# lab-incert/peba1

Measured on AMD Instinct MI355X. Metric: bootstrapped gates/sec (blind rotations/s) over the PEBA1 match path, and end-to-end match ms, higher is better.
Workload: dtype u32

## Files before the change

### peba1_amd/csrc/kernels.hip

```cpp
#include <type_traits>

#include "kernels.hpp"
#include "ntt_wave.hpp"

namespace tfhe_hip {

namespace {

__device__ __forceinline__ PrimeCtx make_ctx(int q, const uint32_t *tw, int n_ring) {
    PrimeCtx c;
    c.P = q ? NTT_P1 : NTT_P0;
    c.pinv = q ? NTT_PINV1 : NTT_PINV0;
    c.rmod = q ? NTT_R[1] : NTT_R[0];
    c.wf = tw + (size_t)(q * 2 + 0) * n_ring;
    c.wi = tw + (size_t)(q * 2 + 1) * n_ring;
    const uint4 *quads = reinterpret_cast<const uint4 *>(tw + (size_t)4 * n_ring);
    c.qf = quads + (size_t)(q * 2 + 0) * (n_ring / 2);
    c.qi = quads + (size_t)(q * 2 + 1) * (n_ring / 2);
    c.dtab = nullptr;
    c.fw1 = nullptr;
    c.fw2 = nullptr;
    return c;
}

// ... 10 lines not shown
    for (int r = 0; r < REGS; ++r) y[r] = mont_redc(acc[r], c.P, c.pinv);
    WaveNtt<LOGN>::inverse(y, c, scr, lane);
}

template <int LOGN>
__global__ __launch_bounds__(64) void bk_transform_kernel(const int32_t *__restrict__ raw, uint32_t *__restrict__ img,
                                                          const uint32_t *__restrict__ tw, int nw,
                                                          uint32_t scale0, uint32_t scale1) {
    using NTT = WaveNtt<LOGN>;
    constexpr int N = NTT::N, REGS = NTT::REGS;
    __shared__ __align__(16) uint32_t scr[NTT::SCRATCH_WORDS];
    const int lane = threadIdx.x;
    const int q = blockIdx.y;
    const int poly = blockIdx.x;
    const int X = poly / nw, w = poly % nw;
    const PrimeCtx c = make_ctx(q, tw, N);
    const uint32_t scale = q ? scale1 : scale0;
    const int32_t *src = raw + (size_t)poly * N;
    int32_t x[REGS];
#pragma unroll
    for (int r = 0; r < REGS; ++r) x[r] = src[r * 64 + lane] % (int32_t)c.P;
    NTT::forward(x, c, scr, lane);
    uint4 *dst = reinterpret_cast<uint4 *>(img + ((size_t)(X * 2 + q) * nw + w) * N) + lane;
#pragma unroll
    for (int g = 0; g < REGS / 4; ++g) {
        uint32_t v[4];
#pragma unroll
        for (int e = 0; e < 4; ++e) {
            int32_t m = x[4 * g + e] % (int32_t)c.P;
            if (m < 0) m += (int32_t)c.P;
            v[e] = (uint32_t)((uint64_t)(uint32_t)m * scale % c.P);
        }
        dst[g * 64] = make_uint4(v[0], v[1], v[2], v[3]);
    }
}

template <int LOGN>
__global__ __launch_bounds__(128) void negacyclic_kernel(const int32_t *__restrict__ ip, const uint32_t *__restrict__ img,
                                                         const uint32_t *__restrict__ tw, int32_t *__restrict__ res) {
    using NTT = WaveNtt<LOGN>;
    constexpr int N = NTT::N, REGS = NTT::REGS;
    __shared__ __align__(16) uint32_t lds_scr[2][NTT::SCRATCH_WORDS];
    const int tid = threadIdx.x;
    const int q = __builtin_amdgcn_readfirstlane(tid >> 6);
    const int lane = tid & 63;
    const PrimeCtx c = make_ctx(q, tw, N);
    uint32_t *scr = lds_scr[q];
    const int32_t *src = ip + (size_t)blockIdx.x * N;
    int32_t x[REGS];
#pragma unroll
    for (int r = 0; r < REGS; ++r) x[r] = src[r * 64 + lane];
    NTT::forward(x, c, scr, lane);
    const uint4 *bp = reinterpret_cast<const uint4 *>(img + (size_t)(blockIdx.x * 2 + q) * N) + lane;
    int64_t acc[REGS];
#pragma unroll
    for (int g = 0; g < REGS / 4; ++g) {
        const uint4 b = bp[g * 64];
        acc[4 * g + 0] = (int64_t)x[4 * g + 0] * (int32_t)b.x;
        acc[4 * g + 1] = (int64_t)x[4 * g + 1] * (int32_t)b.y;
        acc[4 * g + 2] = (int64_t)x[4 * g + 2] * (int32_t)b.z;
        acc[4 * g + 3] = (int64_t)x[4 * g + 3] * (int32_t)b.w;
    }
    int32_t y[REGS];
    finish_inverse<LOGN>(acc, y, c, scr, lane);
#pragma unroll
    for (int r = 0; r < REGS; ++r) scr[r * 64 + lane] = (uint32_t)y[r];
    __syncthreads();
    if (q == 0) {
        const uint32_t *oscr = lds_scr[1];
#pragma unroll
        for (int r = 0; r < REGS; ++r)
            res[(size_t)blockIdx.x * N + r * 64 + lane] = (int32_t)crt_signed_to_torus(y[r], (int32_t)oscr[r * 64 + lane]);
    }
}

template <int LOGN, int THREADS>
__device__ __forceinline__ void prelude_modswitch(const DevParams &p, const RotDesc &rd, const int32_t *__restrict__ pool,
                                                  uint16_t *lds_bar, int tid) {
    const int32_t *A = pool + (size_t)rd.slot_a * p.ct_stride;
    const int32_t *B = pool + (size_t)rd.slot_b * p.ct_stride;
    if (rd.slot_c < 0) {
        for (int i = tid; i <= p.n; i += THREADS) {
            uint32_t t = (uint32_t)rd.sa * (uint32_t)A[i] + (uint32_t)rd.sb * (uint32_t)B[i];
            if (i == p.n) t += (uint32_t)rd.c0;
            lds_bar[i] = (uint16_t)((t + (1u << (30 - LOGN))) >> (31 - LOGN));
        }
    } else {
        const int32_t *C = pool + (size_t)rd.slot_c * p.ct_stride;
        for (int i = tid; i <= p.n; i += THREADS) {
            uint32_t t = (uint32_t)rd.sa * (uint32_t)A[i] + (uint32_t)rd.sb * (uint32_t)B[i] + (uint32_t)rd.sc * (uint32_t)C[i];
            if (i == p.n) t += (uint32_t)rd.c0;
            lds_bar[i] = (uint16_t)((t + (1u << (30 - LOGN))) >> (31 - LOGN));
        }
    }
}

struct ClockProbe {
    unsigned long long c0 = 0, r0 = 0;
    bool on = false;
    __device__ __forceinline__ void begin(const DevParams &p) {
        on = p.clock_acc != nullptr && blockIdx.x % 61 == 0 && threadIdx.x == 0;
        if (on) { c0 = __builtin_amdgcn_s_memtime(); r0 = __builtin_amdgcn_s_memrealtime(); }
    }
    __device__ __forceinline__ void end(const DevParams &p) {
        if (on) {
            atomicAdd(&p.clock_acc[0], __builtin_amdgcn_s_memtime() - c0);
            atomicAdd(&p.clock_acc[1], __builtin_amdgcn_s_memrealtime() - r0);
        }
    }
};

template <int LOGN>
__device__ __forceinline__ uint32_t testvector_coef(int j, int barb, int32_t mu) {
    constexpr int N = 1 << LOGN;
    const int idx = (j + barb) & (2 * N - 1);
    return (idx & N) ? (uint32_t)(-mu) : (uint32_t)mu;
}

template <int LOGN>
__device__ __forceinline__ uint32_t lut_coef(const int32_t *__restrict__ v, int j, int barb) {
    constexpr int N = 1 << LOGN;
    const int idx = (j + barb) & (2 * N - 1);
    const uint32_t w = (uint32_t)v[idx & (N - 1)];
    return (idx & N) ? 0u - w : w;
}

__device__ __forceinline__ const int32_t *lut_of(const DevParams &p, const RotDesc &rd) {
    return rd.lut >= 0 ? p.luts + (size_t)rd.lut * LUT_STRIDE : nullptr;
}

template <int LOGN>
__device__ __forceinline__ uint32_t body_coef(const int32_t *__restrict__ lut, int j, int barb, int32_t mu) {
    return lut ? lut_coef<LOGN>(lut, j, barb) : testvector_coef<LOGN>(j, barb, mu);
}

template <int LOGN>
struct AccLds {
    static constexpr int N = 1 << LOGN;
    uint32_t w[2][3 * N];
    __device__ __forceinline__ void set(int u, int j, uint32_t v) {
        w[u][j] = v; w[u][N + j] = 0u - v; w[u][2 * N + j] = v;
    }
    __device__ __forceinline__ uint32_t get(int u, int j) const { return w[u][j]; }
    template <int REGS>
    __device__ __forceinline__ void rotated_difference(uint32_t (&D)[REGS], int u, int lane, int abar, uint32_t offset) const {
        const uint32_t base = (uint32_t)(lane - abar) & (uint32_t)(2 * N - 1);
        const uint32_t *own_neg = w[u] + N + lane;
        const uint32_t *rot = w[u] + base;
#pragma unroll
        for (int r = 0; r < REGS; ++r) D[r] = (rot[r * 64] + own_neg[r * 64] + offset) ^ offset;
    }
};

template <int LOGN, bool FRESH, bool TABLE, bool LDSTW = false, bool PROGRESS = false, int V = 0>
__device__ __forceinline__ void forward_poly(const DevParams &p, const DevKey &key, const PrimeCtx &c,
                                             const AccLds<LOGN> &lds_acc, uint32_t *scr,
                                             int lane, int q, int i, int u, int abar, bool swap_outputs,
                                             int64_t (&acc0)[WaveNtt<LOGN>::REGS], int64_t (&acc1)[WaveNtt<LOGN>::REGS],
                                             const typename WaveNtt<LOGN>::FwdTw0 &t0, int jbegin = 0, int jend = -1) {
    using NTT = WaveNtt<LOGN>;
    constexpr int N = NTT::N, REGS = NTT::REGS, G4 = REGS / 4;
    uint32_t Dk[REGS];
    lds_acc.template rotated_difference<REGS>(Dk, u, lane, abar, p.decomp_offset);
    const int o0 = swap_outputs ? N / 4 : 0, o1 = N / 4 - o0;
    const int width = p.Bgbit;
    auto row = [&](int jj, auto first) {
        const int prow = u * p.l + jj;
        const uint4 *bp = reinterpret_cast<const uint4 *>(
                              key.bk_img + ((size_t)((size_t)i * p.kpl + prow) * 2 + q) * 2 * N) + lane;
        uint4 b0[G4], b1[G4];
#pragma unroll
        for (int g = 0; g < G4; ++g) b0[g] = bp[o0 + g * 64];
#pragma unroll
        for (int g = 0; g < G4; ++g) b1[g] = bp[o1 + g * 64];
        const int shift = 32 - (jj + 1) * width;
        int32_t x[REGS];
        NTT::template forward_digits<TABLE, LDSTW>(x, Dk, shift, width, c, scr, lane, t0);
#pragma unroll
        for (int g = 0; g < G4; ++g) {
            const int32_t bb0[4] = {(int32_t)b0[g].x, (int32_t)b0[g].y, (int32_t)b0[g].z, (int32_t)b0[g].w};
#pragma unroll
            for (int e = 0; e < 4; ++e) {
                const int r = 4 * g + e;
                if constexpr (decltype(first)::value) acc0[r] = (int64_t)x[r] * bb0[e];
                else acc0[r] += (int64_t)x[r] * bb0[e];
            }
        }
#pragma unroll
        for (int g = 0; g < G4; ++g) {
            const int32_t bb1[4] = {(int32_t)b1[g].x, (int32_t)b1[g].y, (int32_t)b1[g].z, (int32_t)b1[g].w};
#pragma unroll
            for (int e = 0; e < 4; ++e) {
                const int r = 4 * g + e;
                if constexpr (decltype(first)::value) acc1[r] = (int64_t)x[r] * bb1[e];
                else acc1[r] += (int64_t)x[r] * bb1[e];
            }
        }
    };
    if (jend < 0) jend = p.l;
    row(jbegin, std::integral_constant<bool, FRESH>{});
#pragma unroll 1
    for (int jj = jbegin + 1; jj < jend; ++jj) {
        if constexpr (PROGRESS) {
            if (jj == jbegin + 1) __builtin_amdgcn_s_setprio(1);
            else __builtin_amdgcn_s_setprio(2);
        }
        row(jj, std::false_type{});
    }
}

template <int LOGN, int THREADS, typename AccT>
__device__ __forceinline__ void extract_outputs(const DevParams &p, const RotDesc &rd, const AccT &acc,
                                                int32_t *__restrict__ u_buf, int tid) {
    constexpr int N = 1 << LOGN;
    const ExtractSpec &xs = p.specs[rd.spec & XS_ENTRY_MASK];
    const int wanted = rd.spec >> XS_WANTED_SHIFT, nout = xs.nout;
    for (int m = 0; m < nout; ++m) {
        if (!((wanted >> m) & 1)) continue;
        int32_t *u = u_buf + (size_t)(rd.u_index + m) * p.u_stride;
        const int nt = xs.ntaps[m];
        for (int i = tid; i < N; i += THREADS) {
            uint32_t sum = 0;
            for (int t = 0; t < nt; ++t) {
                const int d = xs.index[m][t] - i;
                const uint32_t a = acc.get(0, d & (N - 1));
                sum += (uint32_t)xs.weight[m][t] * (d < 0 ? 0u - a : a);
            }
            u[i] = (int32_t)sum;
        }
        if (tid == 0) {
            uint32_t b = (uint32_t)xs.out_c0[m];
            for (int t = 0; t < nt; ++t) b += (uint32_t)xs.weight[m][t] * acc.get(1, xs.index[m][t]);
            u[N] = (int32_t)b;
        }
    }
}

template <int LOGN, int THREADS, typename AccT>
__device__ __forceinline__ void extract_sample(const DevParams &p, const RotDesc &rd,
                                               const AccT &acc,
                                               int32_t *__restrict__ u_buf, int32_t *__restrict__ acc_dbg, int tid) {
    constexpr int N = 1 << LOGN;
    if (rd.spec >= 0) {
        extract_outputs<LOGN, THREADS>(p, rd, acc, u_buf, tid);
    } else {
        int32_t *u = u_buf + (size_t)rd.u_index * p.u_stride;
        for (int j = tid; j < N; j += THREADS)
            u[j] = (int32_t)(j == 0 ? acc.get(0, 0) : 0u - acc.get(0, N - j));
        if (tid == 0) u[N] = (int32_t)acc.get(1, 0);
    }
    if (acc_dbg) {
        int32_t *d = acc_dbg + (size_t)blockIdx.x * 2 * N;
        for (int j = tid; j < 2 * N; j += THREADS) d[j] = (int32_t)acc.get(j >> LOGN, j & (N - 1));
    }
}

template <int LOGN>
__global__ __launch_bounds__(128) void blind_rotate2_kernel(DevParams p, DevKey key, const int32_t *__restrict__ pool,
                                                           const RotDesc *__restrict__ rots,
                                                           int32_t *__restrict__ u_buf, int32_t *__restrict__ acc_dbg) {
    using NTT = WaveNtt<LOGN>;
    constexpr int N = NTT::N, REGS = NTT::REGS;
    __shared__ __align__(16) AccLds<LOGN> lds_acc;
    __shared__ __align__(16) uint32_t lds_scr[2][NTT::SCRATCH_WORDS];
    __shared__ uint16_t lds_bar[1024 + 8];

    const int tid = threadIdx.x;
    const int q = __builtin_amdgcn_readfirstlane(tid >> 6);
    const int lane = tid & 63;
    const PrimeCtx c = make_ctx(q, key.tw, N);
    uint32_t *scr = lds_scr[q];
    const RotDesc rd = rots[blockIdx.x];
    const int n = p.n;

    prelude_modswitch<LOGN, 128>(p, rd, pool, lds_bar, tid);
    __syncthreads();
    {
        const int barb = lds_bar[n];
        const int32_t *lut = lut_of(p, rd);
#pragma unroll
        for (int r = 0; r < REGS; ++r) {
            const int j = r * 64 + lane;
            lds_acc.set(q, j, q == 0 ? 0u : body_coef<LOGN>(lut, j, barb, p.mu));
        }
    }
    __syncthreads();

    typename NTT::FwdTw0 t0;
    t0.load(c, lane);
    for (int i = 0; i < n; ++i) {
        const int abar = __builtin_amdgcn_readfirstlane((int)lds_bar[i]);
        if (abar == 0) continue;

        int64_t acc0[REGS], acc1[REGS];
        forward_poly<LOGN, true, false>(p, key, c, lds_acc, scr, lane, q, i, 0, abar, false, acc0, acc1, t0);
        forward_poly<LOGN, false, false>(p, key, c, lds_acc, scr, lane, q, i, 1, abar, false, acc0, acc1, t0);

        int32_t y0[REGS], y1[REGS];
        finish_inverse<LOGN>(acc0, y0, c, scr, lane);
        finish_inverse<LOGN>(acc1, y1, c, scr, lane);

        const uint32_t *oscr = lds_scr[1 - q];
        if (q == 0) {
#pragma unroll
            for (int r = 0; r < REGS; ++r) scr[r * 64 + lane] = (uint32_t)y1[r];
            __syncthreads();
#pragma unroll
            for (int r = 0; r < REGS; ++r)
                lds_acc.set(0, r * 64 + lane, lds_acc.get(0, r * 64 + lane) + crt_signed_to_torus(y0[r], (int32_t)oscr[r * 64 + lane]));
        } else {
#pragma unroll
            for (int r = 0; r < REGS; ++r) scr[r * 64 + lane] = (uint32_t)y0[r];
            __syncthreads();
#pragma unroll
            for (int r = 0; r < REGS; ++r)
                lds_acc.set(1, r * 64 + lane, lds_acc.get(1, r * 64 + lane) + crt_signed_to_torus((int32_t)oscr[r * 64 + lane], y1[r]));
        }
        __syncthreads();
    }
    extract_sample<LOGN, 128>(p, rd, lds_acc, u_buf, acc_dbg, tid);
}

#ifdef TFHE_HIP_STAMPS
__device__ unsigned long long g_stamps[8][8];
#define STAMP_DECL unsigned long long st_prev = __builtin_amdgcn_s_memtime(), st_sum[8] = {0, 0, 0, 0, 0, 0, 0, 0}
#define STAMP(k)                                                             \
    do {                                                                     \
        __builtin_amdgcn_sched_barrier(0);                                   \
        const unsigned long long st_now = __builtin_amdgcn_s_memtime();      \
        __builtin_amdgcn_s_waitcnt(0xC07F);                                  \
        st_sum[k] += st_now - st_prev;                                       \
        st_prev = st_now;                                                    \
        __builtin_amdgcn_sched_barrier(0);                                   \
    } while (0)
#define STAMP_FLUSH                                                          \
    do {                                                                     \
        if (lane == 0)                                                       \
            for (int k = 0; k < 8; ++k) atomicAdd(&g_stamps[wv][k], st_sum[k]); \
    } while (0)
#else
#define STAMP_DECL
#define STAMP(k)
#define STAMP_FLUSH
#endif

template <int LOGN>
struct Br4Lds {
    using NTT = WaveNtt<LOGN>;
    AccLds<LOGN> acc;
    uint32_t buf0[4][NTT::SCRATCH_WORDS];
    uint32_t buf1[4][NTT::ROW_WORDS];
    uint16_t bar[1024 + 8];
    alignas(8) uint32_t dtab[2][5 * DIGIT_TAB];
    uint4 ft1[2][64 >> NTT::LC][NTT::FwdTw1::IMAGE16];
    uint4 ft2[2][64][NTT::FwdTw2::IMAGE16];
    __device__ __forceinline__ uint32_t *scr(int wv) { return buf0[wv]; }
    __device__ __forceinline__ uint32_t *x1(int wv) { return buf1[wv]; }
    __device__ __forceinline__ uint32_t *x2(int wv) { return buf0[wv]; }
};
static_assert(sizeof(Br4Lds<10>) <= 80 * 1024, "two workgroups of the 4-wave form must fit the 160 KB of a CU");

template <int LOGN, bool TAB, int V = 0>
__device__ __forceinline__ void blind_rotate4_body(const DevParams &p, const DevKey &key,
                                                   const int32_t *__restrict__ pool, const RotDesc &rd,
                                                   Br4Lds<LOGN> &sh, int tid) {
    using NTT = WaveNtt<LOGN>;
    constexpr int N = NTT::N, REGS = NTT::REGS, HALF = REGS / 2;
    const int wv = __builtin_amdgcn_readfirstlane(tid >> 6);
    const int q = wv & 1, u = wv >> 1;
    const int lane = tid & 63;
    PrimeCtx c = make_ctx(q, key.tw, N);
    uint32_t *scr = sh.scr(wv);
    const int n = p.n;

    prelude_modswitch<LOGN, 256>(p, rd, pool, sh.bar, tid);
    if constexpr (TAB) {
        NTT::build_digit_table(sh.dtab[q], c, p.Bgbit, (u << 6) | lane, 128);
        c.dtab = sh.dtab[q];
    }
    if (u == 0) {
        typename NTT::FwdTw1 a;
        a.load(c, lane);
        if ((lane & ((1 << NTT::LC) - 1)) == 0) a.to_image(sh.ft1[q][lane >> NTT::LC]);
        typename NTT::FwdTw2 b;
        b.load(c, lane);
        b.to_image(sh.ft2[q][lane]);
    }
    c.fw1 = sh.ft1[q][lane >> NTT::LC];
    c.fw2 = sh.ft2[q][lane];
    __syncthreads();
    if (q == 0) {
        const int barb = sh.bar[n];
        const int32_t *lut = lut_of(p, rd);
#pragma unroll
        for (int r = 0; r < REGS; ++r) {
            const int j = r * 64 + lane;
            sh.acc.set(u, j, u == 0 ? 0u : body_coef<LOGN>(lut, j, barb, p.mu));
        }
    }
    __syncthreads();

    STAMP_DECL;
    typename NTT::FwdTw0 t0;
    t0.load(c, lane);

    for (int i = 0; i < n; ++i) {
        const int abar = __builtin_amdgcn_readfirstlane((int)sh.bar[i]);
        if (abar == 0) continue;
        STAMP(0);

        int64_t acc0[REGS], acc1[REGS];
        forward_poly<LOGN, true, TAB, true, true, V>(p, key, c, sh.acc, scr, lane, q, i, u, abar, u != 0, acc0, acc1, t0);
        STAMP(1);

        int32_t t[REGS];
        {
            int32_t send[REGS];
#pragma unroll
            for (int r = 0; r < REGS; ++r) {
                t[r] = mont_redc(acc0[r], c.P, c.pinv);
                send[r] = mont_redc(acc1[r], c.P, c.pinv);
            }
            NTT::write_row(send, sh.x1(wv), lane);
        }
        typename NTT::InvTw2 t2;
        t2.load(c, lane);
        STAMP(2);
        lds_barrier();
        __builtin_amdgcn_s_setprio(3);
        STAMP(3);
        {
            int32_t other[REGS];
            NTT::read_row(other, sh.x1(wv ^ 2), lane);
#pragma unroll
            for (int r = 0; r < REGS; ++r) t[r] += other[r];
        }
        typename NTT::InvTw0 ti0;
        NTT::inverse_head(t, c, scr, lane, t2, ti0);
        STAMP(4);

        const uint32_t *ox = sh.x2(wv ^ 1);
        uint32_t *mx = sh.x2(wv);
        if (q == 0) {
            NTT::template inverse_last<true>(t, c, ti0, [&] {
#pragma unroll
                for (int r = 0; r < HALF; ++r) mx[r * 64 + lane] = (uint32_t)t[HALF + r];
            });
            LDS_BARRIER_ROLE("q=0");
#pragma unroll
            for (int r = 0; r < HALF; ++r)
                sh.acc.set(u, r * 64 + lane, sh.acc.get(u, r * 64 + lane) + crt_signed_to_torus(t[r], (int32_t)ox[r * 64 + lane]));
        } else {
            NTT::template inverse_last<false>(t, c, ti0, [&] {
#pragma unroll
                for (int r = 0; r < HALF; ++r) mx[r * 64 + lane] = (uint32_t)t[r];
            });
            LDS_BARRIER_ROLE("q=1");
#pragma unroll
            for (int r = 0; r < HALF; ++r)
                sh.acc.set(u, (HALF + r) * 64 + lane,
                           sh.acc.get(u, (HALF + r) * 64 + lane) + crt_signed_to_torus((int32_t)ox[r * 64 + lane], t[HALF + r]));
        }
        STAMP(5);
        __builtin_amdgcn_s_setprio(0);
        lds_barrier();
        STAMP(6);
    }
    STAMP_FLUSH;
}

template <int LOGN, bool TAB>
__global__ __launch_bounds__(256, 2) void blind_rotate4_kernel(
    DevParams p, DevKey key, const int32_t *__restrict__ pool, const RotDesc *__restrict__ rots,
    int32_t *__restrict__ u_buf, int32_t *__restrict__ acc_dbg) {
    __shared__ __align__(16) Br4Lds<LOGN> sh;
    if (p.wg_times && threadIdx.x == 0) {
        const uint64_t hw = __builtin_amdgcn_s_getreg((31 << 11) | (0 << 6) | 4);
        const uint64_t xcc = __builtin_amdgcn_s_getreg((3 << 11) | (0 << 6) | 20);
        p.wg_times[4 * blockIdx.x] = (__builtin_amdgcn_s_memtime() & 0xFFFFFFFFFFFFull) |
                                     ((((xcc & 0xF) << 8) | ((hw >> 8) & 0xFF)) << 48);
        p.wg_times[4 * blockIdx.x + 2] = __builtin_amdgcn_s_memrealtime();
    }
    ClockProbe clk;
    clk.begin(p);
    const RotDesc rd = rots[blockIdx.x];
    blind_rotate4_body<LOGN, TAB>(p, key, pool, rd, sh, threadIdx.x);
    extract_sample<LOGN, 256>(p, rd, sh.acc, u_buf, acc_dbg, threadIdx.x);
    clk.end(p);
    if (p.wg_times && threadIdx.x == 0) {
        p.wg_times[4 * blockIdx.x + 1] = __builtin_amdgcn_s_memtime();
        p.wg_times[4 * blockIdx.x + 3] = __builtin_amdgcn_s_memrealtime();
    }
}

__device__ __forceinline__ uint32_t split_finish(int h, int32_t a0, int32_t a1, int32_t b0, int32_t b1, uint32_t iw1_0,
                                                 uint32_t iw1_1) {
    if (h == 0) return crt_signed_to_torus(a0 + a1, b0 + b1);
    return crt_signed_to_torus(mont_mul(a0 - a1, iw1_0, NTT_P0, NTT_PINV0), mont_mul(b0 - b1, iw1_1, NTT_P1, NTT_PINV1));
}

template <int LOGN>
struct Br8Lds {
    using NTT = WaveNtt<LOGN>;
    AccLds<LOGN> acc;
    static_assert(WaveNtt<LOGN - 1>::SCRATCH_WORDS <= NTT::ROW_WORDS, "the half transform's scratch fits the full-size rows");
    uint32_t scr[8][NTT::ROW_WORDS];
    uint32_t pa0[4][NTT::ROW_WORDS];
    uint32_t pa1[4][NTT::ROW_WORDS];
    uint32_t pb0[4][NTT::ROW_WORDS];
    uint32_t pb[4][NTT::ROW_WORDS];
    uint16_t bar[1024 + 8];
    alignas(8) uint32_t dtab[2][5 * DIGIT_TAB];
    uint4 ft1[2][64 >> NTT::LC][NTT::FwdTw1::IMAGE16];
    uint4 ft2[2][64][NTT::FwdTw2::IMAGE16];
};

template <int LOGN, bool TAB>
__global__ __launch_bounds__(512, 2) void blind_rotate8_kernel(
    DevParams p, DevKey key, const int32_t *__restrict__ pool, const RotDesc *__restrict__ rots,
    int32_t *__restrict__ u_buf, int32_t *__restrict__ acc_dbg) {
    __shared__ __align__(16) Br8Lds<LOGN> sh;
#define BR8_TAG 0
#include "br8_body.inc"
#undef BR8_TAG
}

template <int LOGN, bool TAB>
__global__ __launch_bounds__(256, 2) void blind_rotate4_mk_kernel(
    DevParams p, DevKey key, const DevKey *__restrict__ keys, const int32_t *__restrict__ rot_keys,
    const int32_t *__restrict__ pool, const RotDesc *__restrict__ rots, int32_t *__restrict__ u_buf) {
    __shared__ __align__(16) Br4Lds<LOGN> sh;
    ClockProbe clk;
    clk.begin(p);
    const RotDesc rd = rots[blockIdx.x];
    DevKey k = key;
    k.bk_img = keys[__builtin_amdgcn_readfirstlane(rot_keys[blockIdx.x])].bk_img;
    blind_rotate4_body<LOGN, TAB, 1>(p, k, pool, rd, sh, threadIdx.x);
    extract_sample<LOGN, 256>(p, rd, sh.acc, u_buf, nullptr, threadIdx.x);
    clk.end(p);
}

template <int LOGN, bool TAB>
__global__ __launch_bounds__(512, 2) void blind_rotate8_mk_kernel(
    DevParams p, DevKey key, const DevKey *__restrict__ keys, const int32_t *__restrict__ rot_keys,
    const int32_t *__restrict__ pool, const RotDesc *__restrict__ rots, int32_t *__restrict__ u_buf) {
    __shared__ __align__(16) Br8Lds<LOGN> sh;
    int32_t *const acc_dbg = nullptr;
    {
        const DevKey key0 = key;
        DevKey key = key0;
        key.bk_img = keys[__builtin_amdgcn_readfirstlane(rot_keys[blockIdx.x])].bk_img;
#define BR8_TAG 1
#include "br8_body.inc"
#undef BR8_TAG
    }
}

constexpr int SPLIT_TAB2_BITS = 6;
template <int LOGN, int TM>
struct BrSplitLds {
    using SUB = WaveNtt<LOGN - 1>;
    AccLds<LOGN> acc;
    uint32_t scr[8][SUB::SCRATCH_WORDS];
    uint32_t x1[8][SUB::ROW_WORDS];
    uint16_t bar[1024 + 8];
    alignas(8) uint32_t tab[2][2][TM == 2 ? 11 << SPLIT_TAB2_BITS : DIGIT_TAB];
    static constexpr bool LTW = LOGN == 11;
    uint4 ft1[LTW ? 2 : 1][LTW ? 2 : 1][LTW ? (64 >> SUB::LC) : 1][SUB::FwdTw1::IMAGE16];
    uint4 ft2[LTW ? 2 : 1][LTW ? 2 : 1][LTW ? 64 : 1][SUB::FwdTw2::IMAGE16];
};
static_assert(sizeof(BrSplitLds<11, 2>) <= 160 * 1024, "the N = 2048 split form must fit a CU's LDS");

template <int LOGN, int TM>
__global__ __launch_bounds__(512, (LOGN == 10 ? 4 : 2)) void blind_rotate_split_kernel(
    DevParams p, DevKey key, const int32_t *__restrict__ pool, const RotDesc *__restrict__ rots,
    int32_t *__restrict__ u_buf, int32_t *__restrict__ acc_dbg) {
    using SUB = WaveNtt<LOGN - 1>;
    constexpr int N = 1 << LOGN, M = N / 2, RS = SUB::REGS, RF = 2 * RS, G4 = RS / 4, QUARTER = RS / 4;
    __shared__ __align__(16) BrSplitLds<LOGN, TM> sh;
    constexpr bool TAB = TM == 1;
    const int tid = threadIdx.x;
    const int wv = __builtin_amdgcn_readfirstlane(tid >> 6);
    const int q = wv & 1, u = (wv >> 1) & 1, h = wv >> 2;
    const int lane = tid & 63;
    PrimeCtx c = make_sub_ctx(q, h, key.tw, N);
    constexpr bool LTW = BrSplitLds<LOGN, TM>::LTW;
    uint32_t *scr = sh.scr[wv];
    const int n = p.n;
    const RotDesc rd = rots[blockIdx.x];
    const uint32_t w1 = key.tw[(size_t)(q * 2 + 0) * N + 1];
    const uint32_t iw1_0 = key.tw[(size_t)1 * N + 1], iw1_1 = key.tw[(size_t)3 * N + 1];
// ... 686 lines not shown
```

### peba1_amd/csrc/ntt_wave.hpp

```cpp
#pragma once
#include <hip/hip_runtime.h>
#include <stdint.h>

#include "ntt_field.hpp"

namespace tfhe_hip {

struct PrimeCtx {
    uint32_t P;
    uint32_t pinv;
    uint32_t rmod;
    const uint32_t *__restrict__ wf;
    const uint32_t *__restrict__ wi;
    const uint4 *__restrict__ qf;
    const uint4 *__restrict__ qi;
    const uint32_t *dtab;
    const void *fw1, *fw2;
};

constexpr int DIGIT_TAB_BITS = 7, DIGIT_TAB = 1 << DIGIT_TAB_BITS;
constexpr int DIGIT_TAB_MIN_SHIFT = 3;
#ifndef BR_TAB_GROUPS
#define BR_TAB_GROUPS 99
#endif
// ... 128 lines not shown
        return h_addr(j >> RB, j & (REGS - 1));
    }
    static __device__ __forceinline__ int h_t1_addr(int lane, int reg) {
        return h_addr((reg << LC) | (lane & ((1 << LC) - 1)), lane >> LC);
    }
    template <typename T>
    static __device__ __forceinline__ void write_row(const T (&x)[REGS], uint32_t *scr, int lane) {
        uint4 *p = reinterpret_cast<uint4 *>(scr + row_base(lane));
#pragma unroll
        for (int g = 0; g < REGS / 4; ++g)
            p[g] = make_uint4((uint32_t)x[4 * g], (uint32_t)x[4 * g + 1], (uint32_t)x[4 * g + 2], (uint32_t)x[4 * g + 3]);
    }

    template <int CNT>
    static __device__ __forceinline__ void load_tw(uint32_t (&t)[CNT], const uint32_t *__restrict__ w) {
        if constexpr (CNT == 1) {
            t[0] = w[0];
        } else if constexpr (CNT == 2) {
            const uint2 v = *reinterpret_cast<const uint2 *>(w);
            t[0] = v.x; t[1] = v.y;
        } else {
#pragma unroll
            for (int g = 0; g < CNT / 4; ++g) {
                const uint4 v = reinterpret_cast<const uint4 *>(w)[g];
                t[4 * g] = v.x; t[4 * g + 1] = v.y; t[4 * g + 2] = v.z; t[4 * g + 3] = v.w;
            }
        }
    }

    static constexpr int rbit_of(int S) { return S < RB ? RB - 1 - S : S < 2 * RB ? 2 * RB - 1 - S : LOGN - 1 - S; }
    static constexpr int pass_end(int S) { return S < RB ? RB : S < 2 * RB ? 2 * RB : LOGN; }
    static constexpr int pass_begin(int S) { return S < RB ? 0 : S < 2 * RB ? RB : 2 * RB; }
    template <int S>
    static __device__ __forceinline__ int tw_base(int lane) {
        if constexpr (S < RB) return 1 << S;
        else if constexpr (S < 2 * RB) return (1 << S) + ((lane >> LC) << (S - RB));
        else return (1 << S) + (lane << (S - 6));
    }
    template <int CNT>
    static __device__ __forceinline__ void load_quads(uint4 (&q)[CNT], const uint4 *__restrict__ tab) {
#pragma unroll
        for (int e = 0; e < CNT; ++e) q[e] = tab[e];
    }

    template <int S, int END, bool FWD>
    struct PassTw {
        static constexpr bool PAIR = FWD ? (S + 1 < END) : (END - 2 >= S);
        static constexpr int STAGE = FWD ? S : (PAIR ? END - 2 : END - 1);
        static constexpr int CNT = REGS >> (rbit_of(STAGE) + 1);
        uint32_t tw[CNT];
        uint4 q[PAIR ? CNT : 1];
        PassTw<FWD ? S + (PAIR ? 2 : 1) : S, FWD ? END : END - (PAIR ? 2 : 1), FWD> rest;
        __device__ __forceinline__ void load(const PrimeCtx &c, int lane) {
            const int base = tw_base<STAGE>(lane);
            load_tw<CNT>(tw, (FWD ? c.wf : c.wi) + base);
            if constexpr (PAIR) load_quads<CNT>(q, (FWD ? c.qf : c.qi) + base);
            rest.load(c, lane);
        }
        static constexpr int TW16 = (CNT + 3) / 4;
        static constexpr int IMAGE16 = TW16 + (PAIR ? CNT : 0) + decltype(rest)::IMAGE16;
        __device__ __forceinline__ void to_image(uint4 *img) const {
#pragma unroll
            for (int g = 0; g < TW16; ++g)
                img[g] = make_uint4(tw[4 * g], 4 * g + 1 < CNT ? tw[4 * g + 1] : 0u, 4 * g + 2 < CNT ? tw[4 * g + 2] : 0u,
                                    4 * g + 3 < CNT ? tw[4 * g + 3] : 0u);
            if constexpr (PAIR) {
#pragma unroll
                for (int e = 0; e < CNT; ++e) img[TW16 + e] = q[e];
            }
            rest.to_image(img + TW16 + (PAIR ? CNT : 0));
        }
        __device__ __forceinline__ void from_image(const uint4 *img) {
#pragma unroll
            for (int g = 0; g < TW16; ++g) {
                const uint4 v = img[g];
                tw[4 * g] = v.x;
                if constexpr (CNT > 1) { if (4 * g + 1 < CNT) tw[4 * g + 1] = v.y; if (4 * g + 2 < CNT) tw[4 * g + 2] = v.z; if (4 * g + 3 < CNT) tw[4 * g + 3] = v.w; }
            }
            if constexpr (PAIR) {
#pragma unroll
                for (int e = 0; e < CNT; ++e) q[e] = img[TW16 + e];
            }
            rest.from_image(img + TW16 + (PAIR ? CNT : 0));
        }
    };
    template <int S, bool FWD>
    struct PassTw<S, S, FWD> {
        static constexpr int IMAGE16 = 0;
        __device__ __forceinline__ void load(const PrimeCtx &, int) {}
        __device__ __forceinline__ void to_image(uint4 *) const {}
        __device__ __forceinline__ void from_image(const uint4 *) {}
    };
    using FwdTw0 = PassTw<0, RB, true>;
    using FwdTw1 = PassTw<RB, 2 * RB, true>;
    using FwdTw2 = PassTw<2 * RB, LOGN, true>;
    using InvTw2 = PassTw<2 * RB, LOGN, false>;
    using InvTw1 = PassTw<RB, 2 * RB, false>;
    using InvTw0 = PassTw<0, RB, false>;

    template <int STAGE, bool PAIR, bool FWD, bool RENORM, int CNT>
    static __device__ __forceinline__ void step(int32_t (&x)[REGS], const uint32_t (&tw)[CNT], const uint4 *q,
                                                const PrimeCtx &c) {
        constexpr int RBIT = rbit_of(STAGE), h = 1 << RBIT, l = h >> 1;
        static_assert(CNT == (REGS >> (RBIT + 1)), "twiddle count of the step");
        if constexpr (PAIR) {
            static_assert(pass_end(STAGE) == pass_end(STAGE + 1), "a radix-4 step stays inside one pass");
#pragma unroll
            for (int r = 0; r < REGS; ++r)
                if (!(r & (h | l))) {
                    const int e = r >> (RBIT + 1);
                    if constexpr (FWD) ct_bfly4(x[r], x[r | l], x[r | h], x[r | h | l], tw[e], q[e], c);
                    else gs_bfly4<RENORM>(x[r], x[r | l], x[r | h], x[r | h | l], tw[e], q[e], c);
                }
        } else {
#pragma unroll
            for (int r = 0; r < REGS; ++r)
                if (!(r & h)) {
                    if constexpr (FWD) ct_bfly(x[r], x[r | h], tw[r >> (RBIT + 1)], c);
                    else gs_bfly<RENORM>(x[r], x[r | h], tw[r >> (RBIT + 1)], c);
                }
        }
    }
    template <int S, int END>
    static __device__ __forceinline__ void fwd_pass(int32_t (&x)[REGS], const PrimeCtx &c, const PassTw<S, END, true> &t) {
        using T = PassTw<S, END, true>;
        step<T::STAGE, T::PAIR, true, false, T::CNT>(x, t.tw, t.q, c);
        if constexpr (S + (T::PAIR ? 2 : 1) < END) fwd_pass(x, c, t.rest);
    }
    template <int K, int S, int END>
    static __device__ __forceinline__ void inv_pass(int32_t (&x)[REGS], const PrimeCtx &c, const PassTw<S, END, false> &t) {
        using T = PassTw<S, END, false>;
        constexpr InvPlan plan = make_inv_plan(LOGN);
        static_assert(plan.fan[K] == (T::PAIR ? 4 : 2), "plan and pass structure agree");
        step<T::STAGE, T::PAIR, false, plan.renorm[K], T::CNT>(x, t.tw, t.q, c);
        if constexpr (END - (T::PAIR ? 2 : 1) > S) inv_pass<K + 1>(x, c, t.rest);
    }
    static constexpr int steps_in(int stages) { return (stages + 1) / 2; }

    template <bool LDSTW = false>
    static __device__ __forceinline__ void forward(int32_t (&x)[REGS], const PrimeCtx &c, uint32_t *scr, int lane,
                                                   const FwdTw0 &t0) {
        fwd_pass(x, c, t0);
        forward_tail<LDSTW>(x, c, scr, lane);
    }
    static __device__ __forceinline__ void forward(int32_t (&x)[REGS], const PrimeCtx &c, uint32_t *scr, int lane) {
        FwdTw0 t0;
        t0.load(c, lane);
        forward<false>(x, c, scr, lane, t0);
    }

    template <bool TABLE, bool LDSTW = false>
    static __device__ __forceinline__ void forward_digits(int32_t (&x)[REGS], const uint32_t (&D)[REGS], int shift, int width,
                                                          const PrimeCtx &c, uint32_t *scr, int lane, const FwdTw0 &t0) {
        if constexpr (!TABLE) {
#pragma unroll
            for (int r = 0; r < REGS; ++r) x[r] = __builtin_amdgcn_sbfe((int32_t)D[r], shift, width);
            fwd_pass(x, c, t0);
            forward_tail<LDSTW>(x, c, scr, lane);
        } else {
            static_assert(FwdTw0::PAIR && FwdTw0::CNT == 1, "the first step is a radix-4 step with one block");
            constexpr int RBIT = rbit_of(0), h = 1 << RBIT, l = h >> 1;
            const uint32_t mask4 = ((1u << width) - 1u) << 2;
            const int sh = shift - 2;
            const char *tab = reinterpret_cast<const char *>(c.dtab);
            const uint32_t mask8 = mask4 << 1;
            const int sh8 = shift - 3;
            const char *tab1 = tab + DIGIT_TAB * 4, *tab3 = tab + 3 * DIGIT_TAB * 4;
#pragma unroll
            for (int r = 0; r < REGS; ++r)
                if (!(r & (h | l))) {
                    if ((r & (l - 1)) + ((r >> (RBIT + 1)) * l) >= BR_TAB_GROUPS) {
                        x[r] = __builtin_amdgcn_sbfe((int32_t)D[r], shift, width);
                        x[r | l] = __builtin_amdgcn_sbfe((int32_t)D[r | l], shift, width);
                        x[r | h] = __builtin_amdgcn_sbfe((int32_t)D[r | h], shift, width);
                        x[r | h | l] = __builtin_amdgcn_sbfe((int32_t)D[r | h | l], shift, width);
                        ct_bfly4(x[r], x[r | l], x[r | h], x[r | h | l], t0.tw[0], t0.q[0], c);
                        continue;
                    }
                    const int32_t x0 = __builtin_amdgcn_sbfe((int32_t)D[r], shift, width);
                    const uint32_t i1 = (D[r | l] >> sh8) & mask8, i2 = (D[r | h] >> sh) & mask4, i3 = (D[r | h | l] >> sh8) & mask8;
                    const int32_t A = (int32_t)*reinterpret_cast<const uint32_t *>(tab + i2);
                    const uint2 p1 = *reinterpret_cast<const uint2 *>(tab1 + i1), p3 = *reinterpret_cast<const uint2 *>(tab3 + i3);
                    const int32_t S = (int32_t)p1.x + (int32_t)p3.x;
                    const int32_t T = (int32_t)p1.y + (int32_t)p3.y;
                    const int32_t u = x0 + A, v = x0 - A;
                    x[r] = u + S; x[r | l] = u - S; x[r | h] = v + T; x[r | h | l] = v - T;
                }
            forward_rest<LDSTW>(x, c, scr, lane, t0);
        }
    }
    template <bool LDSTW = false>
    static __device__ __forceinline__ void forward_rest(int32_t (&x)[REGS], const PrimeCtx &c, uint32_t *scr, int lane,
                                                        const FwdTw0 &t0) {
        static_assert(FwdTw0::PAIR, "the first step is a radix-4 step");
        if constexpr (RB > 2) fwd_pass(x, c, t0.rest);
        forward_tail<LDSTW>(x, c, scr, lane);
    }
    template <bool LDSTW>
    static __device__ __forceinline__ void forward_tail(int32_t (&x)[REGS], const PrimeCtx &c, uint32_t *scr, int lane) {
        FwdTw1 t1;
        if constexpr (LDSTW) t1.from_image(static_cast<const uint4 *>(c.fw1)); else t1.load(c, lane);
#pragma unroll
        for (int r = 0; r < REGS; ++r) scr[t1_l0_addr(lane, r)] = (uint32_t)x[r];
        wave_lds_fence();
        read_row(x, scr, lane);
        wave_lds_fence();
        fwd_pass(x, c, t1);
        FwdTw2 t2;
        if constexpr (LDSTW) t2.from_image(static_cast<const uint4 *>(c.fw2)); else t2.load(c, lane);
#pragma unroll
        for (int r = 0; r < REGS; ++r) scr[t2_l1_addr(lane, r)] = (uint32_t)x[r];
        wave_lds_fence();
        read_row(x, scr, lane);
        wave_lds_fence();
        fwd_pass(x, c, t2);
    }
    static __device__ __forceinline__ void build_digit_table(uint32_t *tab, const PrimeCtx &c, int width, int tid, int nthreads) {
        const uint4 q = c.qf[1];
        const uint32_t w[5] = {c.wf[1], q.x, q.z, q.y, q.w};
        const int fields = 1 << width;
        for (int e = tid; e < 5 * fields; e += nthreads) {
            const int k = e >> width, f = e & (fields - 1);
            const int32_t d = f < fields / 2 ? f : f - fields;
            const int pos = k == 0 ? f : (k & 1 ? DIGIT_TAB : 3 * DIGIT_TAB) + 2 * f + (k > 2 ? 1 : 0);
            tab[pos] = (uint32_t)mont_mul(d, w[k], c.P, c.pinv);
        }
    }

    template <bool LAYOUT_H = true>
    static __device__ __forceinline__ void inverse(int32_t (&x)[REGS], const PrimeCtx &c, uint32_t *scr, int lane,
                                                   const InvTw2 &t2) {
        inv_pass<0>(x, c, t2);
        InvTw1 t1;
        t1.load(c, lane);
        if constexpr (LAYOUT_H) write_row_h(x, scr, lane); else write_row(x, scr, lane);
        wave_lds_fence();
#pragma unroll
        for (int r = 0; r < REGS; ++r) x[r] = (int32_t)scr[LAYOUT_H ? h_t2_addr(lane, r) : t2_l1_addr(lane, r)];
        wave_lds_fence();
        inv_pass<steps_in(LC)>(x, c, t1);
        InvTw0 t0;
        t0.load(c, lane);
        if constexpr (LAYOUT_H) write_row_h(x, scr, lane); else write_row(x, scr, lane);
        wave_lds_fence();
#pragma unroll
        for (int r = 0; r < REGS; ++r) x[r] = (int32_t)scr[LAYOUT_H ? h_t1_addr(lane, r) : t1_l0_addr(lane, r)];
        wave_lds_fence();
        inv_pass<steps_in(LC) + steps_in(RB)>(x, c, t0);
    }
    static __device__ __forceinline__ void inverse_head(int32_t (&x)[REGS], const PrimeCtx &c, uint32_t *scr, int lane,
                                                        const InvTw2 &t2, InvTw0 &t0) {
        inv_pass<0>(x, c, t2);
        InvTw1 t1;
        t1.load(c, lane);
        write_row_h(x, scr, lane);
        wave_lds_fence();
#pragma unroll
        for (int r = 0; r < REGS; ++r) x[r] = (int32_t)scr[h_t2_addr(lane, r)];
        wave_lds_fence();
        inv_pass<steps_in(LC)>(x, c, t1);
        t0.load(c, lane);
        write_row_h(x, scr, lane);
        wave_lds_fence();
#pragma unroll
        for (int r = 0; r < REGS; ++r) x[r] = (int32_t)scr[h_t1_addr(lane, r)];
        wave_lds_fence();
        inv_pass_head<steps_in(LC) + steps_in(RB)>(x, c, t0);
    }
    template <bool UPPER_FIRST, typename EMIT>
    static __device__ __forceinline__ void inverse_last(int32_t (&x)[REGS], const PrimeCtx &c, const InvTw0 &t0, EMIT emit) {
        inv_pass_last<steps_in(LC) + steps_in(RB), UPPER_FIRST>(x, c, t0, emit);
    }
    template <int K, int S, int END>
    static __device__ __forceinline__ void inv_pass_head(int32_t (&x)[REGS], const PrimeCtx &c, const PassTw<S, END, false> &t) {
        using T = PassTw<S, END, false>;
        constexpr InvPlan plan = make_inv_plan(LOGN);
        if constexpr (END - (T::PAIR ? 2 : 1) > S) {
            step<T::STAGE, T::PAIR, false, plan.renorm[K], T::CNT>(x, t.tw, t.q, c);
            inv_pass_head<K + 1>(x, c, t.rest);
        }
    }
    template <int K, bool UPPER_FIRST, int S, int END, typename EMIT>
    static __device__ __forceinline__ void inv_pass_last(int32_t (&x)[REGS], const PrimeCtx &c, const PassTw<S, END, false> &t,
                                                         EMIT emit) {
        using T = PassTw<S, END, false>;
        constexpr InvPlan plan = make_inv_plan(LOGN);
        if constexpr (END - (T::PAIR ? 2 : 1) > S) {
            inv_pass_last<K + 1, UPPER_FIRST>(x, c, t.rest, emit);
        } else {
            static_assert(T::PAIR && T::STAGE == 0 && T::CNT == 1 && K == plan.nsteps - 1 && plan.renorm[K],
                          "the last step is one renormalising radix-4 block over the register halves");
            constexpr int h = REGS / 2, l = REGS / 4;
            const uint32_t w1 = t.tw[0];
            const uint4 q = t.q[0];
            int32_t s0[l], s1[l], d0[l], d1[l];
#pragma unroll
            for (int r = 0; r < l; ++r) {
                s0[r] = x[r] + x[r | l]; s1[r] = x[r | h] + x[r | h | l];
                d0[r] = x[r] - x[r | l]; d1[r] = x[r | h] - x[r | h | l];
            }
            auto lower = [&] {
#pragma unroll
                for (int r = 0; r < l; ++r) {
                    x[r] = mont_mul(s0[r] + s1[r], c.rmod, c.P, c.pinv);
                    x[r | l] = mont_mul2(d0[r], q.x, d1[r], q.y, c);
                }
            };
            auto upper = [&] {
#pragma unroll
                for (int r = 0; r < l; ++r) {
                    x[r | h] = mont_mul(s0[r] - s1[r], w1, c.P, c.pinv);
                    x[r | h | l] = mont_mul2(d0[r], q.z, d1[r], q.w, c);
                }
            };
            if constexpr (UPPER_FIRST) { upper(); emit(); lower(); }
            else { lower(); emit(); upper(); }
        }
    }
    static __device__ __forceinline__ void inverse(int32_t (&x)[REGS], const PrimeCtx &c, uint32_t *scr, int lane) {
        InvTw2 t2;
        t2.load(c, lane);
        inverse<true>(x, c, scr, lane, t2);
    }
};

__device__ __forceinline__ uint32_t crt_signed_to_torus(int32_t r0, int32_t r1) {
    const int32_t t = mont_mul(r1 - r0, CRT_P0INV_MONT, NTT_P1, NTT_PINV1);
    return (uint32_t)r0 + NTT_P0 * (uint32_t)t;
}

}
```

Before: 111,600.

## Hold forward twiddles in registers and stage inverse twiddles in LDS

By default, the blind-rotate loop now loads the forward-NTT stage-1 and stage-2 twiddles into registers once, before the loop, instead of re-reading them from an LDS image for every digit row. The LDS space this frees is reused to hold images of the inverse-NTT twiddles. The inverse passes then read these from LDS rather than loading them from global memory on every iteration. The aim is to cut repeated twiddle traffic, at the cost of more live registers across the loop, which can lower occupancy or cause spills.

```diff
diff --git a/peba1_amd/csrc/kernels.hip b/peba1_amd/csrc/kernels.hip
--- a/peba1_amd/csrc/kernels.hip
+++ b/peba1_amd/csrc/kernels.hip
@@ -186,14 +186,28 @@
     }
 };
 
-template <int LOGN, bool FRESH, bool TABLE, bool LDSTW = false, bool PROGRESS = false, int V = 0>
+struct NoHeldTw {};
+template <int LOGN>
+struct HeldTw {
+    typename WaveNtt<LOGN>::FwdTw1 t1;
+    typename WaveNtt<LOGN>::FwdTw2 t2;
+    __device__ __forceinline__ void from_images(const PrimeCtx &c) {
+        t1.from_image(static_cast<const uint4 *>(c.fw1));
+        t2.from_image(static_cast<const uint4 *>(c.fw2));
+    }
+};
+template <int LOGN, bool FRESH, bool TABLE, bool LDSTW = false, bool PROGRESS = false, int V = 0, int HELD = 0>
 __device__ __forceinline__ void forward_poly(const DevParams &p, const DevKey &key, const PrimeCtx &c,
                                              const AccLds<LOGN> &lds_acc, uint32_t *scr,
                                              int lane, int q, int i, int u, int abar, bool swap_outputs,
                                              int64_t (&acc0)[WaveNtt<LOGN>::REGS], int64_t (&acc1)[WaveNtt<LOGN>::REGS],
-                                             const typename WaveNtt<LOGN>::FwdTw0 &t0, int jbegin = 0, int jend = -1) {
+                                             const typename WaveNtt<LOGN>::FwdTw0 &t0, int jbegin = 0, int jend = -1,
+                                             const HeldTw<LOGN> *held = nullptr) {
     using NTT = WaveNtt<LOGN>;
     constexpr int N = NTT::N, REGS = NTT::REGS, G4 = REGS / 4;
+    static_assert(HELD == 0 || LDSTW, "held twiddles come from the LDS image");
+    std::conditional_t<HELD == 1, HeldTw<LOGN>, NoHeldTw> own;
+    if constexpr (HELD == 1) own.from_images(c);
     uint32_t Dk[REGS];
     lds_acc.template rotated_difference<REGS>(Dk, u, lane, abar, p.decomp_offset);
     const int o0 = swap_outputs ? N / 4 : 0, o1 = N / 4 - o0;
@@ -209,7 +223,9 @@
         for (int g = 0; g < G4; ++g) b1[g] = bp[o1 + g * 64];
         const int shift = 32 - (jj + 1) * width;
         int32_t x[REGS];
-        NTT::template forward_digits<TABLE, LDSTW>(x, Dk, shift, width, c, scr, lane, t0);
+        if constexpr (HELD == 1) NTT::template forward_digits<TABLE>(x, Dk, shift, width, c, scr, lane, t0, own.t1, own.t2);
+        else if constexpr (HELD == 2) NTT::template forward_digits<TABLE>(x, Dk, shift, width, c, scr, lane, t0, held->t1, held->t2);
+        else NTT::template forward_digits<TABLE, LDSTW>(x, Dk, shift, width, c, scr, lane, t0);
 #pragma unroll
         for (int g = 0; g < G4; ++g) {
             const int32_t bb0[4] = {(int32_t)b0[g].x, (int32_t)b0[g].y, (int32_t)b0[g].z, (int32_t)b0[g].w};
@@ -378,6 +394,9 @@
 #define STAMP_FLUSH
 #endif
 
+#ifndef BR_HELD_TW
+#define BR_HELD_TW 2
+#endif
 template <int LOGN>
 struct Br4Lds {
     using NTT = WaveNtt<LOGN>;
@@ -386,8 +405,14 @@
     uint32_t buf1[4][NTT::ROW_WORDS];
     uint16_t bar[1024 + 8];
     alignas(8) uint32_t dtab[2][5 * DIGIT_TAB];
+#if BR_HELD_TW == 2
+    uint4 it2[2][64][NTT::InvTw2::IMAGE16];
+    uint4 it1[2][64 >> NTT::LC][NTT::InvTw1::IMAGE16];
+    uint4 it0[2][NTT::InvTw0::IMAGE16];
+#else
     uint4 ft1[2][64 >> NTT::LC][NTT::FwdTw1::IMAGE16];
     uint4 ft2[2][64][NTT::FwdTw2::IMAGE16];
+#endif
     __device__ __forceinline__ uint32_t *scr(int wv) { return buf0[wv]; }
     __device__ __forceinline__ uint32_t *x1(int wv) { return buf1[wv]; }
     __device__ __forceinline__ uint32_t *x2(int wv) { return buf0[wv]; }
@@ -412,6 +437,20 @@
         NTT::build_digit_table(sh.dtab[q], c, p.Bgbit, (u << 6) | lane, 128);
         c.dtab = sh.dtab[q];
     }
+#if BR_HELD_TW == 2
+    if (u == 0) {
+        typename NTT::InvTw2 a;
+        a.load(c, lane);
+        a.to_image(sh.it2[q][lane]);
+        typename NTT::InvTw1 b;
+        b.load(c, lane);
+        if ((lane & ((1 << NTT::LC) - 1)) == 0) b.to_image(sh.it1[q][lane >> NTT::LC]);
+        typename NTT::InvTw0 d;
+        d.load(c, lane);
+        if (lane == 0) d.to_image(sh.it0[q]);
+    }
+    const uint4 *const iw2 = sh.it2[q][lane], *const iw1 = sh.it1[q][lane >> NTT::LC], *const iw0 = sh.it0[q];
+#else
     if (u == 0) {
         typename NTT::FwdTw1 a;
         a.load(c, lane);
@@ -422,6 +461,7 @@
     }
     c.fw1 = sh.ft1[q][lane >> NTT::LC];
     c.fw2 = sh.ft2[q][lane];
+#endif
     __syncthreads();
     if (q == 0) {
         const int barb = sh.bar[n];
@@ -437,6 +477,11 @@
     STAMP_DECL;
     typename NTT::FwdTw0 t0;
     t0.load(c, lane);
+#if BR_HELD_TW == 2
+    HeldTw<LOGN> held;
+    held.t1.load(c, lane);
+    held.t2.load(c, lane);
+#endif
 
     for (int i = 0; i < n; ++i) {
         const int abar = __builtin_amdgcn_readfirstlane((int)sh.bar[i]);
@@ -444,7 +489,13 @@
         STAMP(0);
 
         int64_t acc0[REGS], acc1[REGS];
-        forward_poly<LOGN, true, TAB, true, true, V>(p, key, c, sh.acc, scr, lane, q, i, u, abar, u != 0, acc0, acc1, t0);
+#if BR_HELD_TW == 2
+        forward_poly<LOGN, true, TAB, true, true, V, 2>(p, key, c, sh.acc, scr, lane, q, i, u, abar, u != 0, acc0, acc1, t0,
+                                                        0, -1, &held);
+#else
+        forward_poly<LOGN, true, TAB, true, true, V, BR_HELD_TW>(p, key, c, sh.acc, scr, lane, q, i, u, abar, u != 0, acc0,
+                                                                 acc1, t0);
+#endif
         STAMP(1);
 
         int32_t t[REGS];
@@ -458,7 +509,11 @@
             NTT::write_row(send, sh.x1(wv), lane);
         }
         typename NTT::InvTw2 t2;
+#if BR_HELD_TW == 2
+        t2.from_image(iw2);
+#else
         t2.load(c, lane);
+#endif
         STAMP(2);
         lds_barrier();
         __builtin_amdgcn_s_setprio(3);
@@ -470,7 +525,11 @@
             for (int r = 0; r < REGS; ++r) t[r] += other[r];
         }
         typename NTT::InvTw0 ti0;
+#if BR_HELD_TW == 2
+        NTT::inverse_head(t, c, scr, lane, t2, ti0, iw1, iw0);
+#else
         NTT::inverse_head(t, c, scr, lane, t2, ti0);
+#endif
         STAMP(4);
 
         const uint32_t *ox = sh.x2(wv ^ 1);
diff --git a/peba1_amd/csrc/ntt_wave.hpp b/peba1_amd/csrc/ntt_wave.hpp
--- a/peba1_amd/csrc/ntt_wave.hpp
+++ b/peba1_amd/csrc/ntt_wave.hpp
@@ -304,11 +304,22 @@
     template <bool TABLE, bool LDSTW = false>
     static __device__ __forceinline__ void forward_digits(int32_t (&x)[REGS], const uint32_t (&D)[REGS], int shift, int width,
                                                           const PrimeCtx &c, uint32_t *scr, int lane, const FwdTw0 &t0) {
+        forward_digits_then<TABLE>(x, D, shift, width, c, lane, t0, [&] { forward_tail<LDSTW>(x, c, scr, lane); });
+    }
+    template <bool TABLE>
+    static __device__ __forceinline__ void forward_digits(int32_t (&x)[REGS], const uint32_t (&D)[REGS], int shift, int width,
+                                                          const PrimeCtx &c, uint32_t *scr, int lane, const FwdTw0 &t0,
+                                                          const FwdTw1 &t1, const FwdTw2 &t2) {
+        forward_digits_then<TABLE>(x, D, shift, width, c, lane, t0, [&] { forward_tail(x, c, scr, lane, t1, t2); });
+    }
+    template <bool TABLE, typename TAIL>
+    static __device__ __forceinline__ void forward_digits_then(int32_t (&x)[REGS], const uint32_t (&D)[REGS], int shift, int width,
+                                                               const PrimeCtx &c, int lane, const FwdTw0 &t0, TAIL tail) {
         if constexpr (!TABLE) {
 #pragma unroll
             for (int r = 0; r < REGS; ++r) x[r] = __builtin_amdgcn_sbfe((int32_t)D[r], shift, width);
             fwd_pass(x, c, t0);
-            forward_tail<LDSTW>(x, c, scr, lane);
+            tail();
         } else {
             static_assert(FwdTw0::PAIR && FwdTw0::CNT == 1, "the first step is a radix-4 step with one block");
             constexpr int RBIT = rbit_of(0), h = 1 << RBIT, l = h >> 1;
@@ -338,7 +349,9 @@
                     const int32_t u = x0 + A, v = x0 - A;
                     x[r] = u + S; x[r | l] = u - S; x[r | h] = v + T; x[r | h | l] = v - T;
                 }
-            forward_rest<LDSTW>(x, c, scr, lane, t0);
+            static_assert(FwdTw0::PAIR, "the first step is a radix-4 step");
+            if constexpr (RB > 2) fwd_pass(x, c, t0.rest);
+            tail();
         }
     }
     template <bool LDSTW = false>
@@ -360,6 +373,21 @@
         fwd_pass(x, c, t1);
         FwdTw2 t2;
         if constexpr (LDSTW) t2.from_image(static_cast<const uint4 *>(c.fw2)); else t2.load(c, lane);
+#pragma unroll
+        for (int r = 0; r < REGS; ++r) scr[t2_l1_addr(lane, r)] = (uint32_t)x[r];
+        wave_lds_fence();
+        read_row(x, scr, lane);
+        wave_lds_fence();
+        fwd_pass(x, c, t2);
+    }
+    static __device__ __forceinline__ void forward_tail(int32_t (&x)[REGS], const PrimeCtx &c, uint32_t *scr, int lane,
+                                                        const FwdTw1 &t1, const FwdTw2 &t2) {
+#pragma unroll
+        for (int r = 0; r < REGS; ++r) scr[t1_l0_addr(lane, r)] = (uint32_t)x[r];
+        wave_lds_fence();
+        read_row(x, scr, lane);
+        wave_lds_fence();
+        fwd_pass(x, c, t1);
 #pragma unroll
         for (int r = 0; r < REGS; ++r) scr[t2_l1_addr(lane, r)] = (uint32_t)x[r];
         wave_lds_fence();
@@ -401,17 +429,18 @@
         inv_pass<steps_in(LC) + steps_in(RB)>(x, c, t0);
     }
     static __device__ __forceinline__ void inverse_head(int32_t (&x)[REGS], const PrimeCtx &c, uint32_t *scr, int lane,
-                                                        const InvTw2 &t2, InvTw0 &t0) {
+                                                        const InvTw2 &t2, InvTw0 &t0, const uint4 *img1 = nullptr,
+                                                        const uint4 *img0 = nullptr) {
         inv_pass<0>(x, c, t2);
         InvTw1 t1;
-        t1.load(c, lane);
+        if (img1) t1.from_image(img1); else t1.load(c, lane);
         write_row_h(x, scr, lane);
         wave_lds_fence();
 #pragma unroll
         for (int r = 0; r < REGS; ++r) x[r] = (int32_t)scr[h_t2_addr(lane, r)];
         wave_lds_fence();
         inv_pass<steps_in(LC)>(x, c, t1);
-        t0.load(c, lane);
+        if (img0) t0.from_image(img0); else t0.load(c, lane);
         write_row_h(x, scr, lane);
         wave_lds_fence();
 #pragma unroll
```

Result: faster. 115,100 (median of 6 runs) (+3.2%).
